# TCGGroup/Torch_Detection

Hardware: AMD Instinct MI355X
Metric: images/sec ResNet-50-FPN fwd+bwd 1333x800 (higher is better)
Workload: dtype bf16; 1 GPU; ResNet-50 + FPN(256, 5 levels) forward+backward, 2 x 3x800x1344 (1333x800 zero-padded to /32) per GPU, BN eval (reference default), fixed cotangents, all parameter grads; global_batch=2, parallelism=dp1, weights_static=True

## Files before the change

include/tdn.h:

```cpp
#ifndef TDN_H_
#define TDN_H_

#include <stddef.h>
#include <stdint.h>

#ifdef __cplusplus
extern "C" {
#endif

#define TDN_VERSION 100

enum { TDN_BF16 = 0, TDN_F16 = 1 };

enum {
  TDN_ADD_NONE = 0,
  TDN_ADD_SAME = 1,
  TDN_ADD_UP2X = 2,
  TDN_ADD_SUMPOOL2 = 3
};

typedef struct tdn_epilogue {
  const float* scale;
  const float* shift;
  const void* addend;
// ... 30 lines not shown

int64_t tdn_conv2d_wgrad_workspace(int N, int H, int W, int Cin, int Cout, int k, int stride,
                                    int pad);

int tdn_conv2d_wgrad(const void* x, const void* g, const void* w_fwd, const float* scale,
                     const float* mean, const float* invstd, float* dw, float* dgamma,
                     float* dbeta, float beta, int N, int H, int W, int Cin, int Cout, int k,
                     int stride, int pad, void* workspace, int64_t workspace_bytes, int dtype,
                     void* stream);

enum { TDN_WGRAD_CONV = 0, TDN_WGRAD_STEM = 1, TDN_WGRAD_GCONV = 2 };
typedef struct tdn_wgrad_item {
  const void* x;
  const void* g;
  const void* w_fwd;
  const float* scale;
  const float* mean;
  const float* invstd;
  float* dw;
  float* dgamma;
  float* dbeta;
  float beta;
  int32_t kind;
  int32_t N, H, W;
  int32_t Cin, Cout;
  int32_t k, stride, pad;
  int32_t groups;
  int32_t reserved;
} tdn_wgrad_item;
int64_t tdn_wgrad_group_workspace(const tdn_wgrad_item* items, int n, int dtype);
int tdn_wgrad_group(const tdn_wgrad_item* items, int n, void* workspace, int64_t workspace_bytes, int dtype,
                    void* stream);
int tdn_wgrad_group_plan(const tdn_wgrad_item* items, int n, int dtype, int32_t* per_item, int32_t* totals);

typedef struct tdn_prep_item {
  const float* w;
  void* w_fwd;
  void* w_dgrad;
  const float* gamma;
  const float* beta;
  const float* mean;
  const float* var;
  float* fold;
  int64_t s_o, s_i, s_h, s_w;
  int32_t Cout, Cin, kh, kw;
  float eps;
  int32_t reserved;
} tdn_prep_item;
int tdn_prepare_group(const tdn_prep_item* items, int n, int dtype, void* stream);

typedef struct tdn_bottleneck_args {
  const void* in;
  const void* w1;
  const void* w2;
  const void* w3;
  const float* scale1; const float* shift1;
  const float* scale2; const float* shift2;
  const float* scale3; const float* shift3;
  const void* mask1;
  const void* mask2;
  const void* mask3;
  void* out1;
  void* out2;
  void* out3;
  int32_t N, H, W, C;
  void* bits1;
// ... 242 lines not shown
```

torch_detection_amd/_lib.py:

```python
import ctypes
import os
import threading

import torch

_HERE = os.path.dirname(os.path.abspath(__file__))
LIB_PATH = os.path.join(_HERE, os.path.basename(os.environ.get("TDN_LIB", "") or "libtdn.so"))

TDN_BF16 = 0
TDN_F16 = 1
TDN_F32 = 2
NMS_SEG_MAX = 4096
RPN_MAX_LEVELS = 8
RPN_MAX_NUM = 8192
ROI_MAX_LEVELS = 8
ROI_MAX_OUT = 16
ROI_MAX_SAMPLES = 512
TARGET_MAX_GT = 256
TARGET_MAX_BOXES = 1 << 20
TARGET_MAX_NUM = 8192
ADD_NONE, ADD_SAME, ADD_UP2X, ADD_SUMPOOL2 = 0, 1, 2, 3

c_void_p = ctypes.c_void_p
c_int = ctypes.c_int
# ... 104 lines not shown
                ("scale3", c_void_p), ("shift3", c_void_p),
                ("mask1", c_void_p), ("mask2", c_void_p), ("mask3", c_void_p),
                ("out1", c_void_p), ("out2", c_void_p), ("out3", c_void_p),
                ("N", ctypes.c_int32), ("H", ctypes.c_int32), ("W", ctypes.c_int32), ("C", ctypes.c_int32),
                ("bits1", c_void_p), ("bits2", c_void_p), ("bits3", c_void_p)]


_BA = ctypes.POINTER(BottleneckArgs)


class BottleneckHeadArgs(ctypes.Structure):
    _fields_ = [("b", BottleneckArgs), ("addend", c_void_p), ("wd", c_void_p), ("scale_d", c_void_p),
                ("shift_d", c_void_p)]


_BHA = ctypes.POINTER(BottleneckHeadArgs)

SIGNATURES = {
    "tdn_last_error": (ctypes.c_char_p, []),
    "tdn_version": (c_int, []),
    "tdn_bn_fold": (c_int, [c_void_p] * 4 + [c_float, c_int] + [c_void_p] * 3 + [c_void_p]),
    "tdn_pack_conv_weight": (c_int, [c_void_p, c_i64, c_i64, c_i64, c_i64, c_int, c_int, c_int, c_int,
                                     c_void_p, c_void_p, c_void_p, c_int, c_void_p]),
    "tdn_pack_stem_weight": (c_int, [c_void_p, c_int, c_void_p, c_int, c_void_p]),
    "tdn_prepare_group": (c_int, [_PI, c_int, c_int, c_void_p]),
    "tdn_conv2d_fwd": (c_int, [c_void_p] * 3 + [c_int] * 8 + [_EP, c_int, c_void_p]),
    "tdn_conv2d_dgrad": (c_int, [c_void_p] * 3 + [c_int] * 8 + [_EP, c_int, c_void_p]),
    "tdn_conv2d_wgrad_workspace": (c_i64, [c_int] * 8),
    "tdn_conv2d_wgrad": (c_int, [c_void_p] * 9 + [c_float] + [c_int] * 8 + [c_void_p, c_i64, c_int, c_void_p]),
    "tdn_wgrad_group_workspace": (c_i64, [_WI, c_int, c_int]),
    "tdn_wgrad_group": (c_int, [_WI, c_int, c_void_p, c_i64, c_int, c_void_p]),
    "tdn_wgrad_group_plan": (c_int, [_WI, c_int, c_int, ctypes.POINTER(ctypes.c_int32),
                                     ctypes.POINTER(ctypes.c_int32)]),
    "tdn_stage_image": (c_int, [c_void_p, c_i64, c_i64, c_i64, c_i64, c_int, c_int, c_int, c_void_p, c_int,
                                c_void_p]),
    "tdn_stem_conv_fwd": (c_int, [c_void_p] * 3 + [c_int] * 4 + [_EP, c_int, c_void_p]),
    "tdn_stem_pool_fwd": (c_int, [c_void_p] * 6 + [c_int] * 5 + [c_void_p]),
    "tdn_stem_conv_wgrad_workspace": (c_i64, [c_int] * 4),
    "tdn_stem_conv_wgrad": (c_int, [c_void_p] * 9 + [c_float] + [c_int] * 4 + [c_void_p, c_i64, c_int, c_void_p]),
    "tdn_maxpool3x3s2_fwd": (c_int, [c_void_p] * 3 + [c_int] * 5 + [c_void_p]),
    "tdn_maxpool3x3s2_bwd": (c_int, [c_void_p] * 4 + [c_int] * 5 + [c_void_p]),
    "tdn_maxpool3x3s2_relu_bwd": (c_int, [c_void_p] * 4 + [c_int] * 5 + [c_void_p]),
    "tdn_subsample2_fwd": (c_int, [c_void_p] * 2 + [c_int] * 5 + [c_void_p]),
    "tdn_subsample2_bwd": (c_int, [c_void_p] * 3 + [c_int] * 5 + [c_void_p]),
    "tdn_add_relu_mask": (c_int, [c_void_p] * 4 + [c_i64, c_int, c_void_p]),
    "tdn_clamp_max": (c_int, [c_void_p, c_float, c_i64, c_int, c_void_p]),
    "tdn_act_mask": (c_int, [c_void_p] * 3 + [c_float, c_i64, c_int, c_void_p]),
    "tdn_channel_affine_fwd": (c_int, [c_void_p] * 4 + [c_i64, c_int, c_int, c_int, c_void_p]),
    "tdn_channel_affine_bwd_workspace": (c_i64, [c_i64, c_int]),
    "tdn_channel_affine_bwd": (c_int, [c_void_p] * 8 + [c_float, c_i64, c_int, c_void_p, c_i64, c_int, c_void_p]),
    "tdn_nchw_f32_to_nhwc": (c_int, [c_void_p, c_i64, c_i64, c_i64, c_i64, c_int, c_int, c_int, c_int, c_void_p,
                                     c_int, c_void_p]),
    "tdn_nchw16_to_nhwc": (c_int, [c_void_p, c_i64, c_i64, c_i64, c_i64, c_int, c_int, c_int, c_int, c_void_p,
                                   c_void_p]),
    "tdn_nhwc_to_nchw_f32": (c_int, [c_void_p, c_int, c_int, c_int, c_int, c_void_p, c_int, c_void_p]),
    "tdn_anchor_grid": (c_int, [c_void_p, c_int, c_int, c_int, c_int, c_int, c_int, c_void_p, c_void_p, c_void_p]),
    "tdn_anchor_pyramid": (c_int, [_AL, c_int, c_void_p, c_void_p, c_void_p]),
    "tdn_bbox_iou_pairwise": (c_int, [c_void_p, c_int, c_void_p, c_int, c_void_p, c_void_p]),
    "tdn_nms_workspace": (c_i64, [c_int]),
    "tdn_nms": (c_int, [c_void_p, c_void_p, c_int, c_float, c_void_p, c_void_p, c_void_p, c_void_p, c_i64,
                        c_void_p]),
    "tdn_bbox_normalize": (c_int, [c_void_p, c_i64, ctypes.POINTER(c_float), ctypes.POINTER(c_float), c_void_p]),
    "tdn_bbox_denormalize": (c_int, [c_void_p, c_void_p, c_i64, c_int, ctypes.POINTER(c_float),
                                     ctypes.POINTER(c_float), c_void_p]),
    "tdn_bbox2delta": (c_int, [c_void_p, c_void_p, c_i64, ctypes.POINTER(c_float), ctypes.POINTER(c_float), c_void_p,
                               c_void_p]),
# ... 100 lines not shown
```

torch_detection_amd/csrc/conv_wgrad.hip:

```cpp
#include "common.h"
#include <limits.h>
#include <string.h>
#include <type_traits>
#include <algorithm>
#include <math.h>
#include <mutex>
#include <unordered_map>
#include <vector>

constexpr int WG_MAXI = 26;
constexpr int FIN_MAXI = 30;

struct WgItem {
  const bf16_t* x;
  const bf16_t* g;
  const bf16_t* w_fwd;
  const float* scale;
  float* out;
  float* colsum;
  float* dotpart;
  int Hin, Win, Cpix, Ktap;
  int Ho, Wo, Cout, sa;
  int M, Mchunk, splitk;
  int ntaps, Ktot;
  int tiles_co, tiles_k;
  int tapgen;
  int grouped;
  int direct;
  float beta;
  int reserved;
};

struct WgGroup {
  int nitems, reserved;
  int blk_start[WG_MAXI + 2];
  WgItem it[WG_MAXI];
};
static_assert(sizeof(WgGroup) <= 4096, "kernel-argument block too large");

__device__ __forceinline__ void wg_tap(int tapgen, int t, int& dh, int& dw) {
  const int k = tapgen & 0xff, pad = (tapgen >> 8) & 0xff, dil = (tapgen >> 16) & 0xff;
  if (tapgen >> 24) { dh = t; dw = 0; return; }
  const int kh = t / k, kw = t - kh * k;
  dh = kh * dil - pad;
  dw = kw * dil - pad;
}

__device__ __forceinline__ bool wg_work(int bid, int splitk, int ntiles, int& split, int& tile) {
  if (splitk >= 8) {
    const int xj = bid >> 3;
    split = (bid & 7) + 8 * (xj / ntiles);
    tile = xj - (xj / ntiles) * ntiles;
  } else {
    split = bid / ntiles;
    tile = bid - split * ntiles;
  }
  return split < splitk;
}
static int wg_blocks(int splitk, int ntiles) {
  const int slots = splitk >= 8 ? 8 * ((splitk + 7) / 8) : splitk;
  return (slots * ntiles + 7) & ~7;
}

template <int RB>
__device__ __forceinline__ int tr_swz(int row) {
  if constexpr (RB >= 256) return (row & 3) | (((row >> 3) & 1) << 2);
  else if constexpr (RB == 128) return ((row >> 1) & 1) | (((row >> 3) & 1) << 1);
  else return (row >> 3) & 1;
}

template <int N>
__device__ __forceinline__ void wg_wait_vm_and_barrier() {
  asm volatile("s_waitcnt vmcnt(%0)\n\ts_barrier" ::"n"(N) : "memory");
}

#ifdef TDN_TRACE_BUILD
__device__ unsigned long long* g_wg_trace = nullptr;
__device__ int g_wg_trace_cap = 0;
#define WG_STAMP(slot, val)                                                                        \
  do {                                                                                             \
    if (g_wg_trace && tid == 0 && (int)blockIdx.x < g_wg_trace_cap)                                \
      g_wg_trace[(size_t)blockIdx.x * 8 + (slot)] = (unsigned long long)(val);                     \
  } while (0)
extern "C" int tdn_debug_wgrad_trace(void* buf, int nwg_cap) {
  unsigned long long* b = (unsigned long long*)buf;
  hipError_t e = hipMemcpyToSymbol(HIP_SYMBOL(g_wg_trace), &b, sizeof(b));
  TDN_CHECK(e == hipSuccess, "tdn_debug_wgrad_trace: %s", hipGetErrorString(e));
  e = hipMemcpyToSymbol(HIP_SYMBOL(g_wg_trace_cap), &nwg_cap, sizeof(nwg_cap));
  TDN_CHECK(e == hipSuccess, "tdn_debug_wgrad_trace: %s", hipGetErrorString(e));
  return 0;
}
#else
#define WG_STAMP(slot, val) do { } while (0)
#endif

template <int BMW , int BNW , int WM, int WN, int NST, bool F16>
__global__ __launch_bounds__(WM * WN * 64) void conv_wgrad_group_kernel(const WgGroup grp) {
  extern __shared__ __attribute__((aligned(16))) char smem[];
  constexpr int BKW = 64;
  constexpr int RBG = BMW * 2, RBX = BNW * 2;
  constexpr int G_BYTES = BKW * RBG, X_BYTES = BKW * RBX, STAGE = G_BYTES + X_BYTES;
  constexpr int RPIG = 1024 / RBG, RPIX = 1024 / RBX;
  constexpr int NW = WM * WN;
  constexpr int G_IT = BKW / (RPIG * NW), X_IT = BKW / (RPIX * NW);
  static_assert(G_IT >= 1 && X_IT >= 1, "every wave must issue the same number of loads per stage (counted vmcnt)");
  constexpr int LOADS = G_IT + X_IT;
  static_assert(LOADS * (NST - 2) < 64, "vmcnt immediate out of range");
  constexpr int WTM = BMW / WM, WTN = BNW / WN, FM = WTM / 16, FN = WTN / 16;
  static_assert(FM >= 1 && FN >= 1, "tile too small");
  static_assert((RPIG * NW) % 16 == 0 && (RPIX * NW) % 16 == 0, "loader round must be a multiple of 16 rows");
  static_assert(WN * BMW * 4 <= NST * STAGE, "cross-wave reduction buffer must fit the ring");

  const int tid = threadIdx.x;
  const int lane = tid & 63;
  const int wave = __builtin_amdgcn_readfirstlane(tid >> 6);

  int idx = 0;
#pragma unroll
  for (int i = 1; i < WG_MAXI; ++i) idx += ((int)blockIdx.x >= grp.blk_start[i]) ? 1 : 0;
  const WgItem& p = grp.it[idx];
  const int ntiles = p.tiles_co * p.tiles_k;
  int split, tile;
  if (!wg_work((int)blockIdx.x - grp.blk_start[idx], p.splitk, ntiles, split, tile)) return;
  WG_STAMP(0, __builtin_readcyclecounter());
  WG_STAMP(4, __builtin_amdgcn_s_memrealtime());
  const int tile_co = tile % p.tiles_co, tile_k = tile / p.tiles_co;
  const int co0 = tile_co * BMW;
  const int kt_per_tap = p.Ktap / BNW;
  const int tap_i = tile_k / kt_per_tap;
  const int ci_k = (tile_k - tap_i * kt_per_tap) * BNW;
  const int ci0 = p.grouped ? co0 : ci_k;
  int dh, dw;
  wg_tap(p.tapgen, tap_i, dh, dw);
  const int m_begin = split * p.Mchunk;
  const int m_end = min(p.M, m_begin + p.Mchunk);
  const int Cout = p.Cout, Cpix = p.Cpix, Hin = p.Hin, Win = p.Win, sa = p.sa, Wo = p.Wo, Ho = p.Ho;
  const bf16_t* const gx = p.x;
  const bf16_t* const gg = p.g;

  constexpr int CPRG = RBG / 16, CPRX = RBX / 16;
  const int g_lrow = lane / CPRG, g_pc = lane % CPRG;
  const int x_lrow = lane / CPRX, x_pc = lane % CPRX;
  const int g_row0 = wave * RPIG + g_lrow;
  const int x_row0 = wave * RPIX + x_lrow;
  const int g_src_el = ((((g_pc >> 1) ^ tr_swz<RBG>(g_row0)) << 1) | (g_pc & 1)) * 8;
  const int x_src_el = ((((x_pc >> 1) ^ tr_swz<RBX>(x_row0)) << 1) | (x_pc & 1)) * 8;
  const bf16_t* zero = (const bf16_t*)g_zero_page;

  int xa[X_IT], xb[X_IT], ximg[X_IT];
  const int HoWo = Ho * Wo;
#pragma unroll
  for (int it = 0; it < X_IT; ++it) {
    const int m = m_begin + it * (RPIX * NW) + x_row0;
    const int img = m / HoWo;
    const int rem = m - img * HoWo;
    ximg[it] = img;
// ... 157 lines not shown
      float d = dpart[i];
      d += __shfl_xor(d, 16, 64);
      d += __shfl_xor(d, 32, 64);
      if (grp4 == 0) red[wn * BMW + wm * WTM + i * 16 + fr] = d;
    }
    __syncthreads();
    for (int c = tid; c < BMW; c += NW * 64) {
      float s = red[c];
#pragma unroll
      for (int w = 1; w < WN; ++w) s += red[w * BMW + c];
      p.dotpart[(int64_t)tile_k * Cout + co0 + c] = s;
    }
  }
}

template <bool F16, int WMR = 4>
__global__ __launch_bounds__(WMR * 128) void conv_wgrad9_group_kernel(const WgGroup grp) {
  extern __shared__ __attribute__((aligned(16))) char smem[];
  constexpr int BKW = 64, BMW = 32 * WMR, BNW = 64;
  constexpr int NWV = WMR * 2;
  constexpr int RBG = BMW * 2, RBX = BNW * 2;
  constexpr int CPRG = RBG / 16, RPIG = 64 / CPRG;
  constexpr int XIT = 64 / (NWV * 8);
  static_assert(RPIG * NWV == 32 && XIT >= 1, "loader layout");
  constexpr int G_TILE = BKW * RBG;
  constexpr int XROWS = 72;
  constexpr int X_TILE = XROWS * RBX;
  constexpr int STAGE = G_TILE + 3 * X_TILE;
  constexpr int FM = 2, FN = 2, WN = 2, WTM = 16 * FM, WTN = 16 * FN;
  const int tid = threadIdx.x;
  const int lane = tid & 63;
  const int wave = __builtin_amdgcn_readfirstlane(tid >> 6);

  int idx = 0;
#pragma unroll
  for (int i = 1; i < WG_MAXI; ++i) idx += ((int)blockIdx.x >= grp.blk_start[i]) ? 1 : 0;
  const WgItem& p = grp.it[idx];
  const int ntiles = p.tiles_co * p.tiles_k;
  int split, tile;
  if (!wg_work((int)blockIdx.x - grp.blk_start[idx], p.splitk, ntiles, split, tile)) return;
  const int tile_co = tile % p.tiles_co, tile_ci = tile / p.tiles_co;
  const int co0 = tile_co * BMW, ci0 = tile_ci * BNW;
  const int m_begin = split * p.Mchunk;
  const int pM = p.M;
  const int m_end = min(pM, m_begin + p.Mchunk);
  const int W = p.Wo, H = p.Ho;
  const int Cout = p.Cout, Cpix = p.Cpix;
  const bf16_t* const gx = p.x;
  const bf16_t* const gg = p.g;
  const bf16_t* zero = (const bf16_t*)g_zero_page;

  const int g_lrow = lane / CPRG, g_pc = lane % CPRG;
  const int x_lrow = lane >> 3, x_pc = lane & 7;
  const int g_row0 = wave * RPIG + g_lrow;
  const int x_row0 = wave * 8 + x_lrow;
  const int g_src_el = ((((g_pc >> 1) ^ tr_swz<RBG>(g_row0)) << 1) | (g_pc & 1)) * 8;
  const int x_src_el = ((((x_pc >> 1) ^ tr_swz<RBX>(x_row0)) << 1) | (x_pc & 1)) * 8;
  int xh[XIT + 1], xw[XIT + 1];
#pragma unroll
  for (int it = 0; it <= XIT; ++it) {
    const int q = m_begin + it * (NWV * 8) + x_row0 - 1;
    const int qq = q < 0 ? q + W * H : q;
    xw[it] = qq % W;
    xh[it] = (qq / W) % H;
  }

  auto stage_load = [&](int mt, int s) {
    char* sG = smem + s * STAGE;
    char* sX = sG + G_TILE;
#pragma unroll
    for (int it = 0; it < 2; ++it) {
      const int m = mt + it * 32 + g_row0;
      const bf16_t* src = (m < m_end) ? gg + ((int64_t)m * Cout + co0 + g_src_el) : zero + (g_src_el & 127);
// ... 315 lines not shown
          dw[oidx] = (beta != 0.f) ? beta * dw[oidx] + v : v;
        }
      }
    }
  }
#pragma unroll
  for (int o = 32; o > 0; o >>= 1) dot += __shfl_down(dot, o, 64);
  if ((tid & 63) == 0) red[tid >> 6] = dot;
  __syncthreads();
  if (tid < 64) {
    float cs = 0.f;
    for (int sp = tid; sp < splitk; sp += 64) cs += p.colsum[(int64_t)sp * Cout + co];
#pragma unroll
    for (int o = 32; o > 0; o >>= 1) cs += __shfl_down(cs, o, 64);
    if (tid == 0) {
      const float d = (red[0] + red[1]) + (red[2] + red[3]);
      if (p.dbeta) p.dbeta[co] = (beta != 0.f) ? beta * p.dbeta[co] + cs : cs;
      if (p.mean && p.invstd && p.dgamma) {
        const float dg = (d - p.mean[co] * cs) * p.invstd[co];
        p.dgamma[co] = (beta != 0.f) ? beta * p.dgamma[co] + dg : dg;
      }
    }
  }
}

static int conv_dil(int k, int pad) { return k == 3 ? pad : 1; }
static int conv_out(int H, int k, int stride, int pad) {
  return (H + 2 * pad - (conv_dil(k, pad) * (k - 1) + 1)) / stride + 1;
}

static int env_int(const char* name, int dflt) {
  const char* e = getenv(name);
  return (e && *e) ? atoi(e) : dflt;
}

struct TapShape { int bmw, bnw, wm, wn, nst, per_cu, step_clk; };
static const TapShape kTapShapes[] = {
    {64, 32, 2, 2, 2, 6, 1800},
    {64, 64, 2, 2, 2, 5, 2000},
    {64, 64, 2, 2, 3, 3, 1365},
    {128, 64, 2, 2, 2, 3, 2050},
    {128, 64, 2, 2, 3, 2, 1640},
    {256, 64, 4, 2, 2, 2, 2000},
    {256, 64, 4, 2, 3, 1, 1460},
    {128, 128, 2, 2, 2, 2, 2180},
    {256, 128, 4, 2, 2, 1, 1750},
};
static const int kNumTapShapes = (int)(sizeof(kTapShapes) / sizeof(kTapShapes[0]));
static const int kT9StepClk = 2600;

struct ItemPlan {
  int Hin, Win, Cpix, Ktap, Ho, Wo, Cout, sa, M, ntaps, Ktot, tapgen, grouped, map_mode;
  bool t9_ok, bn;
  int variant;
  int shape;
  int tiles_co, tiles_k, splitk, mchunk, direct, blocks, ndot;
  int step_clk, tmin, slots;
  int64_t off_out, off_colsum, off_dot;
};

static int item_geometry(const tdn_wgrad_item& it, ItemPlan& g) {
  TDN_CHECK(it.x && it.g && it.w_fwd && it.dw, "wgrad item: NULL pointer");
  TDN_CHECK(it.N > 0 && it.H > 0 && it.W > 0, "wgrad item: bad tensor shape N=%d H=%d W=%d", it.N, it.H, it.W);
  g.grouped = 0;
  g.t9_ok = false;
  g.bn = it.mean && it.invstd && it.dgamma;
// ... 30 lines not shown
  g.M = it.N * g.Ho * g.Wo;
  g.Ktot = g.ntaps * g.Ktap;
  return 0;
}

static std::mutex g_plan_mutex;
static std::unordered_map<uint64_t, double> g_plan_cache;

static inline int launch_key(const ItemPlan& g) { return g.variant ? -g.variant : g.shape; }

static void launch_lists(const std::vector<ItemPlan>& plans, std::vector<std::vector<int>>& lists) {
  const int n = (int)plans.size();
  for (int key = -2; key < kNumTapShapes; ++key) {
    std::vector<int> cur;
    for (int i = 0; i < n; ++i) {
      if (launch_key(plans[i]) != key) continue;
      cur.push_back(i);
      if ((int)cur.size() == WG_MAXI) { lists.push_back(cur); cur.clear(); }
    }
    if (!cur.empty()) lists.push_back(cur);
  }
}

static void split_member(ItemPlan& g, int T) {
  const int ksteps = ceil_div(g.M, 64);
  if (T < 1) T = 1;
  int splitk = (ksteps + T / 2) / T;
  if (splitk < 1) splitk = 1;
  if (splitk > 256) splitk = 256;
  if (splitk >= 8) splitk = (splitk + 4) / 8 * 8;
  const int mchunk = ceil_div(ceil_div(g.M, splitk), 64) * 64;
  g.splitk = ceil_div(g.M, mchunk);
  g.mchunk = mchunk;
  g.blocks = wg_blocks(g.splitk, g.tiles_co * g.tiles_k);
}

static double model_group(const std::vector<ItemPlan>& plans, const std::vector<std::vector<int>>& lists) {
  double total = 0.0, slab_bytes = 0.0;
  std::vector<double> heap;
  for (const std::vector<int>& L : lists) {
    const int slots = plans[L[0]].slots;
    heap.assign(slots, 0.0);
    auto cmp = [](double a, double b) { return a > b; };
    double end = 0.0;
    for (int i : L) {
      const ItemPlan& g = plans[i];
      const int tile_floats = g.variant ? 9 * (g.variant == 2 ? 64 : 128) * 64 : kTapShapes[g.shape].bmw * kTapShapes[g.shape].bnw;
      const double c = (double)ceil_div(g.mchunk, 64) * g.step_clk + tile_floats * 4.0 / 20.0 + 3000.0;
      const int live = g.splitk * g.tiles_co * g.tiles_k;
      for (int b = 0; b < live; ++b) {
        std::pop_heap(heap.begin(), heap.end(), cmp);
        const double t = heap.back() + c;
        heap.back() = t;
        std::push_heap(heap.begin(), heap.end(), cmp);
        if (t > end) end = t;
      }
      if (!g.direct) slab_bytes += (double)g.splitk * g.Cout * g.Ktot * 4.0;
    }
    total += end;
  }
  return total + slab_bytes / 4096.0;
}

static int plan_group(const tdn_wgrad_item* items, int n, std::vector<ItemPlan>& plans, int64_t* ws_floats) {
  TDN_CHECK(items != nullptr && n > 0, "wgrad group: no items");
  plans.resize(n);
  const int t9_mode = env_int("TDN_WGRAD9", 1);
  const int t9_64 = env_int("TDN_WGRAD9_64", 1);
  const int shape_env = env_int("TDN_WGRAD_SHAPE", -1);
  const int s256 = env_int("TDN_WGRAD_S256", 8), s128 = env_int("TDN_WGRAD_S128", 4), s64 = env_int("TDN_WGRAD_S64", 2);
  const int s256f = env_int("TDN_WGRAD_S256F", 5);
  const int uniform = env_int("TDN_WGRAD_UNIFORM", 0);
  const int tmin_tap = env_int("TDN_WGRAD_TMIN", 24), tmin_t9 = env_int("TDN_WGRAD9_TMIN", 32);
  const int direct_ok = env_int("TDN_WGRAD_DIRECT", 1);
  int min_bmw = 256;
  for (int i = 0; i < n; ++i) {
    ItemPlan& g = plans[i];
    if (item_geometry(items[i], g)) return -1;
    g.variant = (g.t9_ok && t9_mode != 0) ? (g.Cout % 128 == 0 ? 1 : (t9_64 ? 2 : 0)) : 0;
    if (!g.variant && !g.grouped && g.Ktap != 32) {
      const int b = g.Cout % 256 == 0 ? 256 : (g.Cout % 128 == 0 ? 128 : 64);
      if (b < min_bmw) min_bmw = b;
    }
  }
  for (int i = 0; i < n; ++i) {
    ItemPlan& g = plans[i];
    if (g.variant) {
      g.shape = -1;
      g.tiles_co = g.Cout / (g.variant == 2 ? 64 : 128);
      g.tiles_k = g.Ktap / 64;
      g.step_clk = kT9StepClk;
      g.tmin = tmin_t9;
      g.slots = g.variant == 2 ? 512 : 256;
    } else {
      int bmw = g.Cout % 256 == 0 ? 256 : (g.Cout % 128 == 0 ? 128 : 64);
      if (uniform && bmw > min_bmw) bmw = min_bmw;
      int shape = g.Ktap == 32 ? 0 : ((g.grouped || bmw == 64) ? s64 : (bmw == 128 ? s128 : s256));
      auto fits = [&](int sh) {
        return sh >= 0 && sh < kNumTapShapes && g.Cout % kTapShapes[sh].bmw == 0 && g.Ktap % kTapShapes[sh].bnw == 0 &&
               !(g.grouped && (kTapShapes[sh].bmw != 64 || kTapShapes[sh].bnw != 64));
      };
      if (!fits(shape) && bmw == 256 && !g.grouped && fits(s256f)) shape = s256f;
      if (!fits(shape)) shape = g.Ktap == 32 ? 0 : (g.Ktap % 64 == 0 ? 2 : 0);
      if (shape_env >= 0 && shape_env < kNumTapShapes && !g.grouped && g.Cout % kTapShapes[shape_env].bmw == 0 &&
          g.Ktap % kTapShapes[shape_env].bnw == 0)
        shape = shape_env;
      g.shape = shape;
      const TapShape& s = kTapShapes[shape];
      g.tiles_co = g.Cout / s.bmw;
      g.tiles_k = g.ntaps * (g.Ktap / s.bnw);
      g.step_clk = s.step_clk;
      g.tmin = tmin_tap;
      g.slots = 256 * s.per_cu;
    }
  }
  std::vector<std::vector<int>> lists;
  launch_lists(plans, lists);
  const double dmin = env_int("TDN_WGRAD_DMIN", 40000), dmax = env_int("TDN_WGRAD_DMAX", 400000);
  const int fixed_t = env_int("TDN_WGRAD_T", 0);
  uint64_t key = 1469598103934665603ull;
  auto mix = [&key](int64_t v) { key = (key ^ (uint64_t)v) * 1099511628211ull; };
  mix(n); mix((int64_t)dmin); mix((int64_t)dmax); mix(fixed_t);
  for (const ItemPlan& g : plans) {
    mix(g.M); mix(g.Cout); mix(g.Ktap); mix(g.ntaps); mix(g.variant); mix(g.shape); mix(g.tmin); mix(g.map_mode);
    mix(g.step_clk);
  }
  double best = -1.0, bestD = dmin;
  bool hit = false;
  {
    std::lock_guard<std::mutex> lock(g_plan_mutex);
    auto itc = g_plan_cache.find(key);
    if (itc != g_plan_cache.end()) { bestD = itc->second; hit = true; }
  }
  const int ncand = (fixed_t > 0 || hit) ? 0 : 24;
  for (int c = 0; c < ncand; ++c) {
    const double D = dmin * pow(dmax / dmin, ncand > 1 ? (double)c / (ncand - 1) : 0.0);
    for (ItemPlan& g : plans) {
      int T = fixed_t > 0 ? fixed_t : (int)(D / g.step_clk + 0.5);
      if (T < g.tmin) T = g.tmin;
      split_member(g, T);
      g.direct = (g.splitk == 1 && g.map_mode == 0 && direct_ok) ? 1 : 0;
    }
    const double t = model_group(plans, lists);
    if (best < 0 || t < best) { best = t; bestD = D; }
  }
  if (ncand > 0) {
    std::lock_guard<std::mutex> lock(g_plan_mutex);
    g_plan_cache[key] = bestD;
  }
  int64_t off = 0;
  for (int i = 0; i < n; ++i) {
    ItemPlan& g = plans[i];
    int T = fixed_t > 0 ? fixed_t : (int)(bestD / g.step_clk + 0.5);
    if (T < g.tmin) T = g.tmin;
    split_member(g, T);
    g.direct = (g.splitk == 1 && g.map_mode == 0 && direct_ok) ? 1 : 0;
    g.ndot = (g.direct && g.bn) ? g.tiles_k : 0;
    g.off_out = off;
    if (!g.direct) off += (int64_t)g.splitk * g.Cout * g.Ktot;
    g.off_colsum = off;
    off += (int64_t)g.splitk * g.Cout;
    g.off_dot = off;
    off += (int64_t)g.ndot * g.Cout;
    off = (off + 63) & ~(int64_t)63;
  }
  *ws_floats = off;
  return 0;
}

template <int BMW, int BNW, int WM, int WN, int NST, bool F16>
static int launch_tap_t(const WgGroup& grp, int nblocks, hipStream_t stream) {
  constexpr size_t lds = (size_t)NST * 64 * (BMW + BNW) * 2;
  static tdn_attr_once attr_once;
  if (attr_once.need()) {
    hipError_t e = hipFuncSetAttribute((const void*)conv_wgrad_group_kernel<BMW, BNW, WM, WN, NST, F16>,
                                       hipFuncAttributeMaxDynamicSharedMemorySize, (int)lds);
    TDN_CHECK(e == hipSuccess, "hipFuncSetAttribute(%d B LDS) failed: %s", (int)lds, hipGetErrorString(e));
    attr_once.mark();
  }
  TDN_LAUNCH((conv_wgrad_group_kernel<BMW, BNW, WM, WN, NST, F16>), dim3(nblocks), dim3(WM * WN * 64), lds,
                     stream, grp);
  TDN_LAUNCH_CHECK();
  return 0;
}

template <bool F16>
static int launch_tap(int shape, const WgGroup& grp, int nblocks, hipStream_t stream) {
  switch (shape) {
    case 0: return launch_tap_t<64, 32, 2, 2, 2, F16>(grp, nblocks, stream);
    case 1: return launch_tap_t<64, 64, 2, 2, 2, F16>(grp, nblocks, stream);
    case 2: return launch_tap_t<64, 64, 2, 2, 3, F16>(grp, nblocks, stream);
    case 3: return launch_tap_t<128, 64, 2, 2, 2, F16>(grp, nblocks, stream);
    case 4: return launch_tap_t<128, 64, 2, 2, 3, F16>(grp, nblocks, stream);
    case 5: return launch_tap_t<256, 64, 4, 2, 2, F16>(grp, nblocks, stream);
    case 6: return launch_tap_t<256, 64, 4, 2, 3, F16>(grp, nblocks, stream);
    case 7: return launch_tap_t<128, 128, 2, 2, 2, F16>(grp, nblocks, stream);
    case 8: return launch_tap_t<256, 128, 4, 2, 2, F16>(grp, nblocks, stream);
    default: tdn_set_error("wgrad: bad tile shape id %d", shape); return -1;
  }
}

template <bool F16, int WMR>
static int launch_t9(const WgGroup& grp, int nblocks, hipStream_t stream) {
  constexpr size_t lds = 2 * (size_t)(64 * (64 * WMR) + 3 * 72 * 128);
  static tdn_attr_once attr_once;
  if (attr_once.need()) {
    hipError_t e = hipFuncSetAttribute((const void*)conv_wgrad9_group_kernel<F16, WMR>,
                                       hipFuncAttributeMaxDynamicSharedMemorySize, (int)lds);
    TDN_CHECK(e == hipSuccess, "hipFuncSetAttribute(%d B LDS) failed: %s", (int)lds, hipGetErrorString(e));
    attr_once.mark();
  }
  TDN_LAUNCH((conv_wgrad9_group_kernel<F16, WMR>), dim3(nblocks), dim3(WMR * 128), lds, stream, grp);
  TDN_LAUNCH_CHECK();
  return 0;
}

static void fill_item(WgItem& d, const tdn_wgrad_item& it, const ItemPlan& g, float* ws) {
  memset(&d, 0, sizeof(d));
  d.x = (const bf16_t*)it.x; d.g = (const bf16_t*)it.g; d.w_fwd = (const bf16_t*)it.w_fwd;
  d.scale = it.scale;
  d.out = g.direct ? it.dw : ws + g.off_out;
  d.colsum = ws + g.off_colsum;
  d.dotpart = g.ndot ? ws + g.off_dot : nullptr;
  d.Hin = g.Hin; d.Win = g.Win; d.Cpix = g.Cpix; d.Ktap = g.Ktap; d.Ho = g.Ho; d.Wo = g.Wo; d.Cout = g.Cout;
  d.sa = g.sa; d.M = g.M; d.Mchunk = g.mchunk; d.splitk = g.splitk; d.ntaps = g.ntaps; d.Ktot = g.Ktot;
  d.tiles_co = g.tiles_co; d.tiles_k = g.tiles_k; d.tapgen = g.tapgen; d.grouped = g.grouped; d.direct = g.direct;
  d.beta = it.beta;
}

extern "C" int64_t tdn_wgrad_group_workspace(const tdn_wgrad_item* items, int n, int dtype) {
  if (dtype != TDN_BF16 && dtype != TDN_F16) { tdn_set_error("dtype %d is neither TDN_BF16 nor TDN_F16", dtype); return -1; }
  std::vector<ItemPlan> plans;
  int64_t fl = 0;
  if (plan_group(items, n, plans, &fl)) return -1;
  return fl * 4 + 256;
}

extern "C" int tdn_wgrad_group_plan(const tdn_wgrad_item* items, int n, int dtype, int32_t* per_item,
                                    int32_t* totals) {
  TDN_CHECK(dtype == TDN_BF16 || dtype == TDN_F16, "dtype %d is neither TDN_BF16 nor TDN_F16", dtype);
  std::vector<ItemPlan> plans;
  int64_t fl = 0;
  if (plan_group(items, n, plans, &fl)) return -1;
  std::vector<std::vector<int>> lists;
  launch_lists(plans, lists);
  int64_t blocks = 0, slab_kib = 0;
  for (int i = 0; i < n; ++i) {
    const ItemPlan& g = plans[i];
    const int64_t slab = g.direct ? 0 : (int64_t)g.splitk * g.Cout * g.Ktot * 4 / 1024;
    if (per_item) {
      int32_t* o = per_item + 8 * i;
      o[0] = g.variant; o[1] = g.variant ? (g.variant == 2 ? 64 : 128) : kTapShapes[g.shape].bmw; o[2] = g.variant ? 64 : kTapShapes[g.shape].bnw;
      o[3] = g.splitk; o[4] = g.mchunk; o[5] = g.direct; o[6] = g.blocks; o[7] = (int32_t)slab;
    }
    blocks += g.blocks;
    slab_kib += slab;
  }
  if (totals) {
    totals[0] = (int32_t)lists.size();
    totals[1] = ceil_div(n, FIN_MAXI);
    totals[2] = (int32_t)blocks;
    totals[3] = (int32_t)slab_kib;
  }
  return 0;
}

extern "C" int tdn_wgrad_group(const tdn_wgrad_item* items, int n, void* workspace, int64_t workspace_bytes,
                               int dtype, void* stream_) {
  TDN_CHECK(dtype == TDN_BF16 || dtype == TDN_F16, "dtype %d is neither TDN_BF16 nor TDN_F16", dtype);
  hipStream_t stream = (hipStream_t)stream_;
  std::vector<ItemPlan> plans;
  int64_t fl = 0;
  if (plan_group(items, n, plans, &fl)) return -1;
  TDN_CHECK(workspace != nullptr && workspace_bytes >= fl * 4, "wgrad workspace too small: %lld < %lld",
            (long long)workspace_bytes, (long long)(fl * 4));
  TDN_CHECK(((uintptr_t)workspace & 15) == 0, "wgrad workspace must be 16-byte aligned");
  float* ws = (float*)workspace;
  std::vector<std::vector<int>> lists;
  launch_lists(plans, lists);
  for (const std::vector<int>& L : lists) {
    WgGroup grp;
    memset(&grp, 0, sizeof(grp));
    grp.nitems = (int)L.size();
    grp.reserved = env_int("TDN_WGRAD9_STAGGER", 1);
    int blk = 0;
    for (int j = 0; j < WG_MAXI + 2; ++j) grp.blk_start[j] = INT_MAX;
    for (int j = 0; j < (int)L.size(); ++j) {
      const int i = L[j];
      grp.blk_start[j] = blk;
      fill_item(grp.it[j], items[i], plans[i], ws);
      blk += plans[i].blocks;
    }
    const ItemPlan& g0 = plans[L[0]];
    int rc;
    if (g0.variant == 2) rc = dtype == TDN_F16 ? launch_t9<true, 2>(grp, blk, stream) : launch_t9<false, 2>(grp, blk, stream);
    else if (g0.variant) rc = dtype == TDN_F16 ? launch_t9<true, 4>(grp, blk, stream) : launch_t9<false, 4>(grp, blk, stream);
    else rc = dtype == TDN_F16 ? launch_tap<true>(g0.shape, grp, blk, stream) : launch_tap<false>(g0.shape, grp, blk, stream);
    if (rc) return rc;
  }
  for (int base = 0; base < n; base += FIN_MAXI) {
    FinGroup fg;
    memset(&fg, 0, sizeof(fg));
    const int cnt = (n - base < FIN_MAXI) ? n - base : FIN_MAXI;
    fg.nitems = cnt;
    for (int j = 0; j < FIN_MAXI + 2; ++j) fg.blk_start[j] = INT_MAX;
    int blk = 0;
    for (int j = 0; j < cnt; ++j) {
      const tdn_wgrad_item& it = items[base + j];
      const ItemPlan& g = plans[base + j];
      FinItem& f = fg.it[j];
      fg.blk_start[j] = blk;
      f.slab = g.direct ? nullptr : ws + g.off_out;
      f.colsum = ws + g.off_colsum;
      f.dotpart = g.ndot ? ws + g.off_dot : nullptr;
      f.w_fwd = (const bf16_t*)it.w_fwd;
      f.scale = it.scale; f.mean = it.mean; f.invstd = it.invstd;
      f.dw = it.dw; f.dgamma = it.dgamma; f.dbeta = it.dbeta; f.beta = it.beta;
      f.splitk = g.splitk; f.Cout = g.Cout; f.Ktot = g.Ktot; f.map_mode = g.map_mode; f.ndot = g.ndot;
      int k4p = 1;
      while (k4p < (g.Ktot >> 2) && k4p < 256) k4p <<= 1;
      f.K4P = k4p;
      blk += g.direct ? ceil_div(g.Cout, 256) : g.Cout;
    }
    if (dtype == TDN_F16)
      TDN_LAUNCH(wgrad_finalize_group_kernel<true>, dim3(blk), dim3(256), 0, stream, fg);
// ... 85 lines not shown
```

Measured before the change: 533.0 images/sec.

## Add XCD-aware block-to-work mapping for grouped wgrad launches

Replaces the linear blk_start block-to-item mapping in the grouped weight-gradient kernels with a per-XCD (bid&7) start table. An optional balancing mode groups items that share an input or gradient tensor onto the same XCD rotation and picks rotations to even out modeled load. It also caches environment knobs and adds a map-inspection API. The XCD mapping is off by default (TDN_WGRAD_MAP=0), so the default path only changes the indexing scheme, which now does more per-block work to locate its item.

```diff
diff --git a/include/tdn.h b/include/tdn.h
--- a/include/tdn.h
+++ b/include/tdn.h
@@ -86,6 +86,7 @@
 int tdn_wgrad_group(const tdn_wgrad_item* items, int n, void* workspace, int64_t workspace_bytes, int dtype,
                     void* stream);
 int tdn_wgrad_group_plan(const tdn_wgrad_item* items, int n, int dtype, int32_t* per_item, int32_t* totals);
+int tdn_wgrad_group_map(const tdn_wgrad_item* items, int n, int dtype, int launch, int32_t* rows, int cap_rows);
 
 typedef struct tdn_prep_item {
   const float* w;
diff --git a/torch_detection_amd/_lib.py b/torch_detection_amd/_lib.py
--- a/torch_detection_amd/_lib.py
+++ b/torch_detection_amd/_lib.py
@@ -160,6 +160,7 @@
     "tdn_wgrad_group": (c_int, [_WI, c_int, c_void_p, c_i64, c_int, c_void_p]),
     "tdn_wgrad_group_plan": (c_int, [_WI, c_int, c_int, ctypes.POINTER(ctypes.c_int32),
                                      ctypes.POINTER(ctypes.c_int32)]),
+    "tdn_wgrad_group_map": (c_int, [_WI, c_int, c_int, c_int, ctypes.POINTER(ctypes.c_int32), c_int]),
     "tdn_stage_image": (c_int, [c_void_p, c_i64, c_i64, c_i64, c_i64, c_int, c_int, c_int, c_void_p, c_int,
                                 c_void_p]),
     "tdn_stem_conv_fwd": (c_int, [c_void_p] * 3 + [c_int] * 4 + [_EP, c_int, c_void_p]),
diff --git a/torch_detection_amd/csrc/conv_wgrad.hip b/torch_detection_amd/csrc/conv_wgrad.hip
--- a/torch_detection_amd/csrc/conv_wgrad.hip
+++ b/torch_detection_amd/csrc/conv_wgrad.hip
@@ -33,7 +33,8 @@
 
 struct WgGroup {
   int nitems, reserved;
-  int blk_start[WG_MAXI + 2];
+  int base[WG_MAXI + 1];
+  unsigned off2[WG_MAXI + 1][4];
   WgItem it[WG_MAXI];
 };
 static_assert(sizeof(WgGroup) <= 4096, "kernel-argument block too large");
@@ -46,20 +47,38 @@
   dw = kw * dil - pad;
 }
 
-__device__ __forceinline__ bool wg_work(int bid, int splitk, int ntiles, int& split, int& tile) {
-  if (splitk >= 8) {
-    const int xj = bid >> 3;
-    split = (bid & 7) + 8 * (xj / ntiles);
-    tile = xj - (xj / ntiles) * ntiles;
+__host__ __device__ __forceinline__ int wg_start(const WgGroup& grp, int i, int x) {
+  return grp.base[i] + (int)((grp.off2[i][x >> 1] >> ((x & 1) * 16)) & 0xffffu);
+}
+__host__ __device__ __forceinline__ bool wg_locate(const WgGroup& grp, int bid, int& idx, int& split, int& tile) {
+  const int x = bid & 7, j = bid >> 3;
+  int st = wg_start(grp, 0, x);
+  idx = 0;
+#pragma unroll
+  for (int i = 1; i <= WG_MAXI; ++i) {
+    const int s = wg_start(grp, i, x);
+    const bool hit = j >= s;
+    idx += hit ? 1 : 0;
+    st = hit ? s : st;
+  }
+  if (idx >= grp.nitems) return false;
+  const WgItem& p = grp.it[idx];
+  const int ntiles = p.tiles_co * p.tiles_k;
+  const int l = j - st;
+  if (p.reserved & 0x100) {
+    const int lb = l * 8 + x;
+    split = lb / ntiles;
+    tile = lb - split * ntiles;
   } else {
-    split = bid / ntiles;
-    tile = bid - split * ntiles;
-  }
-  return split < splitk;
-}
-static int wg_blocks(int splitk, int ntiles) {
-  const int slots = splitk >= 8 ? 8 * ((splitk + 7) / 8) : splitk;
-  return (slots * ntiles + 7) & ~7;
+    const int lc = (p.reserved >> 4) & 3;
+    const int tpc = (ntiles + (1 << lc) - 1) >> lc;
+    const int u = l / tpc;
+    const int vs = ((x - p.reserved) & 7) + 8 * u;
+    split = vs >> lc;
+    tile = (vs & ((1 << lc) - 1)) * tpc + (l - u * tpc);
+    if (tile >= ntiles) return false;
+  }
+  return split < p.splitk;
 }
 
 template <int RB>
@@ -115,13 +134,9 @@
   const int lane = tid & 63;
   const int wave = __builtin_amdgcn_readfirstlane(tid >> 6);
 
-  int idx = 0;
-#pragma unroll
-  for (int i = 1; i < WG_MAXI; ++i) idx += ((int)blockIdx.x >= grp.blk_start[i]) ? 1 : 0;
+  int idx, split, tile;
+  if (!wg_locate(grp, (int)blockIdx.x, idx, split, tile)) return;
   const WgItem& p = grp.it[idx];
-  const int ntiles = p.tiles_co * p.tiles_k;
-  int split, tile;
-  if (!wg_work((int)blockIdx.x - grp.blk_start[idx], p.splitk, ntiles, split, tile)) return;
   WG_STAMP(0, __builtin_readcyclecounter());
   WG_STAMP(4, __builtin_amdgcn_s_memrealtime());
   const int tile_co = tile % p.tiles_co, tile_k = tile / p.tiles_co;
@@ -345,13 +360,9 @@
   const int lane = tid & 63;
   const int wave = __builtin_amdgcn_readfirstlane(tid >> 6);
 
-  int idx = 0;
-#pragma unroll
-  for (int i = 1; i < WG_MAXI; ++i) idx += ((int)blockIdx.x >= grp.blk_start[i]) ? 1 : 0;
+  int idx, split, tile;
+  if (!wg_locate(grp, (int)blockIdx.x, idx, split, tile)) return;
   const WgItem& p = grp.it[idx];
-  const int ntiles = p.tiles_co * p.tiles_k;
-  int split, tile;
-  if (!wg_work((int)blockIdx.x - grp.blk_start[idx], p.splitk, ntiles, split, tile)) return;
   const int tile_co = tile % p.tiles_co, tile_ci = tile / p.tiles_co;
   const int co0 = tile_co * BMW, ci0 = tile_ci * BNW;
   const int m_begin = split * p.Mchunk;
@@ -733,6 +744,39 @@
 static int env_int(const char* name, int dflt) {
   const char* e = getenv(name);
   return (e && *e) ? atoi(e) : dflt;
+}
+
+struct WgKnobs {
+  int t9_mode, t9_64, shape_env, s256, s128, s64, s256f, uniform, tmin_tap, tmin_t9, direct_ok, dmin, dmax, fixed_t;
+  int stagger;
+  int xcd_map;
+};
+extern char** environ;
+static WgKnobs wg_knobs() {
+  static std::mutex mu;
+  static uint64_t seen = 0;
+  static bool valid = false;
+  static WgKnobs k;
+  uint64_t h = 1469598103934665603ull;
+  for (char** e = environ; e && *e; ++e) h = (h ^ (uint64_t)(uintptr_t)*e) * 1099511628211ull;
+  std::lock_guard<std::mutex> lock(mu);
+  if (!valid || h != seen) {
+    k.t9_mode = env_int("TDN_WGRAD9", 1);
+    k.t9_64 = env_int("TDN_WGRAD9_64", 1);
+    k.shape_env = env_int("TDN_WGRAD_SHAPE", -1);
+    k.s256 = env_int("TDN_WGRAD_S256", 8); k.s128 = env_int("TDN_WGRAD_S128", 4); k.s64 = env_int("TDN_WGRAD_S64", 2);
+    k.s256f = env_int("TDN_WGRAD_S256F", 5);
+    k.uniform = env_int("TDN_WGRAD_UNIFORM", 0);
+    k.tmin_tap = env_int("TDN_WGRAD_TMIN", 24); k.tmin_t9 = env_int("TDN_WGRAD9_TMIN", 32);
+    k.direct_ok = env_int("TDN_WGRAD_DIRECT", 1);
+    k.dmin = env_int("TDN_WGRAD_DMIN", 40000); k.dmax = env_int("TDN_WGRAD_DMAX", 400000);
+    k.fixed_t = env_int("TDN_WGRAD_T", 0);
+    k.stagger = env_int("TDN_WGRAD9_STAGGER", 1);
+    k.xcd_map = env_int("TDN_WGRAD_MAP", 0);
+    seen = h;
+    valid = true;
+  }
+  return k;
 }
 
 struct TapShape { int bmw, bnw, wm, wn, nst, per_cu, step_clk; };
@@ -829,7 +873,7 @@
   const int mchunk = ceil_div(ceil_div(g.M, splitk), 64) * 64;
   g.splitk = ceil_div(g.M, mchunk);
   g.mchunk = mchunk;
-  g.blocks = wg_blocks(g.splitk, g.tiles_co * g.tiles_k);
+  g.blocks = g.splitk * g.tiles_co * g.tiles_k;
 }
 
 static double model_group(const std::vector<ItemPlan>& plans, const std::vector<std::vector<int>>& lists) {
@@ -862,14 +906,10 @@
 static int plan_group(const tdn_wgrad_item* items, int n, std::vector<ItemPlan>& plans, int64_t* ws_floats) {
   TDN_CHECK(items != nullptr && n > 0, "wgrad group: no items");
   plans.resize(n);
-  const int t9_mode = env_int("TDN_WGRAD9", 1);
-  const int t9_64 = env_int("TDN_WGRAD9_64", 1);
-  const int shape_env = env_int("TDN_WGRAD_SHAPE", -1);
-  const int s256 = env_int("TDN_WGRAD_S256", 8), s128 = env_int("TDN_WGRAD_S128", 4), s64 = env_int("TDN_WGRAD_S64", 2);
-  const int s256f = env_int("TDN_WGRAD_S256F", 5);
-  const int uniform = env_int("TDN_WGRAD_UNIFORM", 0);
-  const int tmin_tap = env_int("TDN_WGRAD_TMIN", 24), tmin_t9 = env_int("TDN_WGRAD9_TMIN", 32);
-  const int direct_ok = env_int("TDN_WGRAD_DIRECT", 1);
+  const WgKnobs kn = wg_knobs();
+  const int t9_mode = kn.t9_mode, t9_64 = kn.t9_64, shape_env = kn.shape_env;
+  const int s256 = kn.s256, s128 = kn.s128, s64 = kn.s64, s256f = kn.s256f, uniform = kn.uniform;
+  const int tmin_tap = kn.tmin_tap, tmin_t9 = kn.tmin_t9, direct_ok = kn.direct_ok;
   int min_bmw = 256;
   for (int i = 0; i < n; ++i) {
     ItemPlan& g = plans[i];
@@ -913,8 +953,8 @@
   }
   std::vector<std::vector<int>> lists;
   launch_lists(plans, lists);
-  const double dmin = env_int("TDN_WGRAD_DMIN", 40000), dmax = env_int("TDN_WGRAD_DMAX", 400000);
-  const int fixed_t = env_int("TDN_WGRAD_T", 0);
+  const double dmin = kn.dmin, dmax = kn.dmax;
+  const int fixed_t = kn.fixed_t;
   uint64_t key = 1469598103934665603ull;
   auto mix = [&key](int64_t v) { key = (key ^ (uint64_t)v) * 1099511628211ull; };
   mix(n); mix((int64_t)dmin); mix((int64_t)dmax); mix(fixed_t);
@@ -965,6 +1005,118 @@
   return 0;
 }
 
+static double wg_cost(const ItemPlan& g) {
+  const int tile_floats = g.variant ? 9 * (g.variant == 2 ? 64 : 128) * 64 : kTapShapes[g.shape].bmw * kTapShapes[g.shape].bnw;
+  return (double)ceil_div(g.mchunk, 64) * g.step_clk + tile_floats * 4.0 / 20.0 + 3000.0;
+}
+
+static bool wg_shares(const tdn_wgrad_item& a, const ItemPlan& ga, const tdn_wgrad_item& b, const ItemPlan& gb) {
+  if (ga.M != gb.M || ga.mchunk != gb.mchunk || ga.splitk != gb.splitk) return false;
+  if (a.g == b.g && ga.Cout == gb.Cout) return true;
+  return a.x == b.x && ga.Hin == gb.Hin && ga.Win == gb.Win && ga.Cpix == gb.Cpix && ga.sa == gb.sa &&
+         ga.Ho == gb.Ho && ga.Wo == gb.Wo;
+}
+
+static int wg_build_map(const tdn_wgrad_item* items, const std::vector<ItemPlan>& plans, const std::vector<int>& L,
+                        bool xcd_map, WgGroup& grp, std::vector<int>& order) {
+  const int n = (int)L.size();
+  order.clear();
+  std::vector<int> lead(n, -1);
+  if (xcd_map) {
+    std::vector<char> used(n, 0);
+    for (int a = 0; a < n; ++a) {
+      if (used[a]) continue;
+      used[a] = 1;
+      const int la = (int)order.size();
+      order.push_back(L[a]);
+      for (int b = a + 1; b < n; ++b) {
+        if (used[b] || !wg_shares(items[L[a]], plans[L[a]], items[L[b]], plans[L[b]])) continue;
+        used[b] = 1;
+        lead[order.size()] = la;
+        order.push_back(L[b]);
+      }
+    }
+  } else {
+    order = L;
+  }
+  int pos[8] = {0, 0, 0, 0, 0, 0, 0, 0};
+  double load[8] = {0, 0, 0, 0, 0, 0, 0, 0};
+  bool fits = true;
+  auto put_start = [&](int j) {
+    int lo = pos[0];
+    for (int x = 1; x < 8; ++x) lo = std::min(lo, pos[x]);
+    grp.base[j] = lo;
+    for (int x = 0; x < 8; ++x) {
+      const int d = pos[x] - lo;
+      if (d > 0xffff) fits = false;
+      grp.off2[j][x >> 1] |= (unsigned)(d & 0xffff) << ((x & 1) * 16);
+    }
+  };
+  for (int j = 0; j <= WG_MAXI; ++j) {
+    grp.base[j] = INT_MAX;
+    for (int w = 0; w < 4; ++w) grp.off2[j][w] = 0;
+  }
+  for (int j = 0; j < n; ++j) {
+    const ItemPlan& g = plans[order[j]];
+    const int ntiles = g.tiles_co * g.tiles_k;
+    put_start(j);
+    if (!xcd_map) {
+      const bool plain = g.splitk < 8;
+      const int npos = plain ? ceil_div(g.splitk * ntiles, 8) : ceil_div(g.splitk, 8) * ntiles;
+      for (int x = 0; x < 8; ++x) pos[x] += npos;
+      grp.it[j].reserved = plain ? 0x100 : 0;
+      continue;
+    }
+    auto chunks_log2 = [](const ItemPlan& h) {
+      const int nt = h.tiles_co * h.tiles_k, cap4 = std::max(1, h.slots / 32);
+      int lc = 0;
+      while (h.splitk < 8 && lc < 3 && ((nt + (1 << lc) - 1) >> lc) > cap4) ++lc;
+      return lc;
+    };
+    auto units_on = [](int nunits, int r) { return r < nunits ? (nunits - r + 7) / 8 : 0; };
+    const int lc = chunks_log2(g);
+    const int tpc = (ntiles + (1 << lc) - 1) >> lc;
+    int rot = 0;
+    if (lead[j] >= 0) {
+      rot = grp.it[lead[j]].reserved & 7;
+    } else {
+      double unit[8] = {0, 0, 0, 0, 0, 0, 0, 0};
+      for (int k = j; k < n; ++k) {
+        if (k != j && lead[k] != j) continue;
+        const ItemPlan& h = plans[order[k]];
+        const int hl = chunks_log2(h);
+        const double c = wg_cost(h) * ((h.tiles_co * h.tiles_k + (1 << hl) - 1) >> hl);
+        for (int r = 0; r < 8; ++r) unit[r] += c * units_on(h.splitk << hl, r);
+      }
+      double best = -1.0, best2 = 0.0;
+      for (int cand = 0; cand < 8; ++cand) {
+        double worst = 0.0, sq = 0.0;
+        for (int x = 0; x < 8; ++x) {
+          const double v = load[x] + unit[(x - cand) & 7];
+          worst = std::max(worst, v);
+          sq += v * v;
+        }
+        if (best < 0 || worst < best || (worst == best && sq < best2)) { best = worst; best2 = sq; rot = cand; }
+      }
+    }
+    const double c = wg_cost(g) * tpc;
+    for (int x = 0; x < 8; ++x) {
+      const int cnt = units_on(g.splitk << lc, (x - rot) & 7);
+      pos[x] += cnt * tpc;
+      load[x] += c * cnt;
+    }
+    grp.it[j].reserved = rot | (lc << 4);
+  }
+  put_start(n);
+  if (!fits && xcd_map) {
+    for (int j = 0; j < n; ++j) grp.it[j].reserved = 0;
+    return wg_build_map(items, plans, L, false, grp, order);
+  }
+  int grid = 0;
+  for (int x = 0; x < 8; ++x) grid = std::max(grid, pos[x]);
+  return grid * 8;
+}
+
 template <int BMW, int BNW, int WM, int WN, int NST, bool F16>
 static int launch_tap_t(const WgGroup& grp, int nblocks, hipStream_t stream) {
   constexpr size_t lds = (size_t)NST * 64 * (BMW + BNW) * 2;
@@ -1025,6 +1177,21 @@
   d.beta = it.beta;
 }
 
+static int wg_fill_group(const tdn_wgrad_item* items, const std::vector<ItemPlan>& plans, const std::vector<int>& L,
+                         float* ws, WgGroup& grp, std::vector<int>& order) {
+  const WgKnobs kn = wg_knobs();
+  memset(&grp, 0, sizeof(grp));
+  grp.nitems = (int)L.size();
+  grp.reserved = kn.stagger;
+  const int blk = wg_build_map(items, plans, L, kn.xcd_map != 0, grp, order);
+  for (int j = 0; j < (int)order.size(); ++j) {
+    const int mode = grp.it[j].reserved;
+    fill_item(grp.it[j], items[order[j]], plans[order[j]], ws);
+    grp.it[j].reserved = mode;
+  }
+  return blk;
+}
+
 extern "C" int64_t tdn_wgrad_group_workspace(const tdn_wgrad_item* items, int n, int dtype) {
   if (dtype != TDN_BF16 && dtype != TDN_F16) { tdn_set_error("dtype %d is neither TDN_BF16 nor TDN_F16", dtype); return -1; }
   std::vector<ItemPlan> plans;
@@ -1042,6 +1209,11 @@
   std::vector<std::vector<int>> lists;
   launch_lists(plans, lists);
   int64_t blocks = 0, slab_kib = 0;
+  for (const std::vector<int>& L : lists) {
+    WgGroup grp;
+    std::vector<int> order;
+    blocks += wg_fill_group(items, plans, L, nullptr, grp, order);
+  }
   for (int i = 0; i < n; ++i) {
     const ItemPlan& g = plans[i];
     const int64_t slab = g.direct ? 0 : (int64_t)g.splitk * g.Cout * g.Ktot * 4 / 1024;
@@ -1050,7 +1222,6 @@
       o[0] = g.variant; o[1] = g.variant ? (g.variant == 2 ? 64 : 128) : kTapShapes[g.shape].bmw; o[2] = g.variant ? 64 : kTapShapes[g.shape].bnw;
       o[3] = g.splitk; o[4] = g.mchunk; o[5] = g.direct; o[6] = g.blocks; o[7] = (int32_t)slab;
     }
-    blocks += g.blocks;
     slab_kib += slab;
   }
   if (totals) {
@@ -1060,6 +1231,28 @@
     totals[3] = (int32_t)slab_kib;
   }
   return 0;
+}
+
+extern "C" int tdn_wgrad_group_map(const tdn_wgrad_item* items, int n, int dtype, int launch, int32_t* rows,
+                                   int cap_rows) {
+  TDN_CHECK(dtype == TDN_BF16 || dtype == TDN_F16, "dtype %d is neither TDN_BF16 nor TDN_F16", dtype);
+  std::vector<ItemPlan> plans;
+  int64_t fl = 0;
+  if (plan_group(items, n, plans, &fl)) return -1;
+  std::vector<std::vector<int>> lists;
+  launch_lists(plans, lists);
+  TDN_CHECK(launch >= 0 && launch < (int)lists.size(), "wgrad map: launch %d of %d", launch, (int)lists.size());
+  WgGroup grp;
+  std::vector<int> order;
+  const int blk = wg_fill_group(items, plans, lists[launch], nullptr, grp, order);
+  for (int b = 0; rows && b < blk && b < cap_rows; ++b) {
+    int idx, split, tile;
+    int32_t* o = rows + 4 * b;
+    o[3] = b & 7;
+    if (wg_locate(grp, b, idx, split, tile)) { o[0] = order[idx]; o[1] = split; o[2] = tile; }
+    else { o[0] = -1; o[1] = o[2] = 0; }
+  }
+  return blk;
 }
 
 extern "C" int tdn_wgrad_group(const tdn_wgrad_item* items, int n, void* workspace, int64_t workspace_bytes,
@@ -1077,17 +1270,8 @@
   launch_lists(plans, lists);
   for (const std::vector<int>& L : lists) {
     WgGroup grp;
-    memset(&grp, 0, sizeof(grp));
-    grp.nitems = (int)L.size();
-    grp.reserved = env_int("TDN_WGRAD9_STAGGER", 1);
-    int blk = 0;
-    for (int j = 0; j < WG_MAXI + 2; ++j) grp.blk_start[j] = INT_MAX;
-    for (int j = 0; j < (int)L.size(); ++j) {
-      const int i = L[j];
-      grp.blk_start[j] = blk;
-      fill_item(grp.it[j], items[i], plans[i], ws);
-      blk += plans[i].blocks;
-    }
+    std::vector<int> order;
+    const int blk = wg_fill_group(items, plans, L, ws, grp, order);
     const ItemPlan& g0 = plans[L[0]];
     int rc;
     if (g0.variant == 2) rc = dtype == TDN_F16 ? launch_t9<true, 2>(grp, blk, stream) : launch_t9<false, 2>(grp, blk, stream);
```

Result: no change. 532.8 images/sec (-0.0%).
